# sdu-hpcl/BGSA

Measured on AMD Instinct MI355X. Metric: GCUPS (cell updates/sec) all-pairs Myers 150bp, higher is better.
Workload: dtype u32

## Files before the change

bgsa_amd/__init__.py:

```python
from __future__ import annotations

import ctypes
import os
import subprocess
from pathlib import Path

import numpy as np

HERE = Path(__file__).resolve().parent
LIB_PATH = Path(os.environ["BGSA_HIP_LIB"]) if os.environ.get("BGSA_HIP_LIB") else HERE / "libbgsa_hip.so"
LIB_AB_PATH = HERE / "libbgsa_hip_ab.so"
INCLUDE = HERE.parent / "include" / "bgsa_hip.h"

ALGO_MYERS, ALGO_BANDED, ALGO_BITPAL = 0, 1, 2
DISTANCE_BEYOND = -2
V_NUM = 64

_lib = None


class Params(ctypes.Structure):
    _fields_ = [("algo", ctypes.c_int), ("alignment", ctypes.c_int), ("match", ctypes.c_int),
                ("mismatch", ctypes.c_int), ("gap", ctypes.c_int), ("k", ctypes.c_int)]

# ... 96 lines not shown
            getattr(L, name).restype = restype
    L.bgsa_hip_stream_faults.argtypes = [i32]
    L.bgsa_hip_debug_inject_stream_fault.argtypes = [i32]
    L.bgsa_hip_set_auto_resident.argtypes = [i32]
    L.bgsa_hip_set_strict_resident.argtypes = [i32]
    L.bgsa_hip_stale_ranges.argtypes = [ctypes.POINTER(ctypes.c_uint64)]
    L.bgsa_hip_bucket_resident.argtypes = [vp, sz, i32]
    L.bgsa_hip_bucket_release.argtypes = [vp]
    u64p = ctypes.POINTER(ctypes.c_uint64)
    L.bgsa_hip_seam_stats.argtypes = [u64p, u64p, u64p]
    L.bgsa_hip_row_cache_stats.argtypes = [u64p, u64p]
    L.bgsa_hip_event_create.argtypes = [ctypes.POINTER(vp)]
    L.bgsa_hip_event_destroy.argtypes = [vp]
    L.bgsa_hip_event_record.argtypes = [vp, vp]
    L.bgsa_hip_event_synchronize.argtypes = [vp]
    L.bgsa_hip_event_elapsed_ms.argtypes = [vp, vp, ctypes.POINTER(ctypes.c_float)]
    L.bgsa_hip_stream_wait_event.argtypes = [vp, vp]
    L.bgsa_hip_query_stream.argtypes = [i32, vp, i32, i32, vp, i32]
    L.bgsa_hip_myers_band_stream.argtypes = [vp, i32, i32, vp, i32]
    L.bgsa_hip_myers_band_half.argtypes = [i32, i32]
    L.bgsa_hip_myers_band_stats.argtypes = [vp, i32]
    if hasattr(L, "bgsa_hip_myers_band_groups"):
        L.bgsa_hip_myers_band_groups.argtypes = [i32, i64, i32, i32, i32]
    L.bgsa_hip_kernel_name.argtypes = [i32, i32]
    L.bgsa_hip_kernel_name.restype = ctypes.c_char_p
    L.bgsa_hip_malloc.argtypes = [ctypes.POINTER(vp), sz]
    L.bgsa_hip_free.argtypes = [vp]
    L.bgsa_hip_malloc_host.argtypes = [ctypes.POINTER(vp), sz]
    L.bgsa_hip_free_host.argtypes = [vp]
    L.bgsa_hip_memcpy_h2d.argtypes = [vp, vp, sz, vp]
    L.bgsa_hip_memcpy_d2h.argtypes = [vp, vp, sz, vp]
    L.bgsa_hip_memset.argtypes = [vp, i32, sz, vp]
    L.bgsa_hip_stream_synchronize.argtypes = [vp]
    L.bgsa_hip_stream_create.argtypes = [ctypes.POINTER(vp)]
    L.bgsa_hip_stream_destroy.argtypes = [vp]
    L.bgsa_hip_set_device.argtypes = [i32]
    L.hip_handle_reads.argtypes = [vp, vp, i32, i64, i64]
    L.hip_handle_reads.restype = None
    L.hip_cal_align_score.argtypes = [vp, vp, vp, i32, i32, i32, i32, i32, i32, i32, i32, vp]
    L.hip_cal_align_score.restype = None
    L.align_hip.argtypes = [vp, vp, i32, i32, i32, i32, i32, vp, vp]
    L.align_hip.restype = None
    L.init_mapping_table.restype = None
    L.malloc_mem.argtypes = [ctypes.c_uint64]
    L.malloc_mem.restype = vp
    L.free_mem.argtypes = [vp]
# ... 726 lines not shown
```

bgsa_amd/csrc/bgsa_common.h:

```cpp
#pragma once

#include <hip/hip_runtime.h>
#include <stdint.h>
#include <stdlib.h>
#include <stdio.h>

#include <type_traits>

#include "../../include/bgsa_hip.h"

namespace bgsa {

constexpr int kLanes = HIP_V_NUM;
constexpr int kChars = BGSA_CHAR_NUM;
constexpr int kWavesPerBlock = 4;
constexpr int kMaxWords = 32;

void set_error(const char *what, hipError_t e, const char *file, int line);
void set_error_text(const char *text);

#define BGSA_HIP_TRY(expr)                                              \
    do {                                                                \
        hipError_t e_ = (expr);                                         \
        if (e_ != hipSuccess) {                                         \
// ... 39 lines not shown
        *n_blocks = (word_num + nw - 1) / nw;
        return nw;
    }
    template <typename F>
    static int dispatch(int nw, const char *family, F &&f)
    {
        int rc = BGSA_HIP_EUNSUPPORTED;
        if (((N == nw ? (rc = f(std::integral_constant<int, N>{}), true) : false) || ...)) return rc;
        char msg[128];
        snprintf(msg, sizeof msg, "%s: no kernel of %d words in this build", family, nw);
        set_error_text(msg);
        return BGSA_HIP_EUNSUPPORTED;
    }
    template <int M>
    constexpr Widths<N..., M> with() const { return {}; }
};
template <typename A, typename B> struct JoinWidths;
template <int... A, int... B> struct JoinWidths<Widths<A...>, Widths<B...>> { using type = Widths<A..., B...>; };
template <typename A, typename B> using Join = typename JoinWidths<A, B>::type;

int launch_myers(const ScoreArgs &a, int semi_global = 0);
const char *myers_kernel_name(int word_num, int semi_global = 0);
int myers_band_groups(int word_num, int64_t read_count, int ref_len, int read_len, int mixed_lengths);

constexpr int kCodeEnd = 5, kCodeRefill = 6;
inline int stream_windows(int ref_len) { return ref_len / 7 + 1; }
inline size_t stream_stride(int ref_len) { return static_cast<size_t>(stream_windows(ref_len) + 1) * 8; }
__host__ __device__ inline unsigned long long plain_stream_window(const char *row, int ref_len, int i)
{
    const int n_windows = ref_len / 7 + 1;
    unsigned long long win = 0;
    for (int j = 0; j < 8; j++) {
        unsigned code = kCodeEnd;
        if (i < n_windows) {
            const int pos = 7 * i + j;
            if (j == 7) code = (i < n_windows - 1) ? kCodeRefill : kCodeEnd;
            else if (pos < ref_len) {
                code = static_cast<unsigned char>(row[pos]);
                if (code > 4) code = 0;
            }
        }
        win |= static_cast<unsigned long long>(code) << (8 * j);
    }
    return win;
}
int launch_pack_queries(const char *d_content, int ref_len, int ref_start, int ref_end,
// ... 424 lines not shown
```

bgsa_amd/csrc/capi.hip:

```cpp
#include <stdlib.h>
#include <string.h>

#include <algorithm>
#include <atomic>
#include <chrono>
#include <map>
#include <memory>
#include <mutex>
#include <string>
#include <thread>
#include <utility>
#include <vector>

#include "bgsa_common.h"
#include "myers_band.h"

namespace bgsa {

static thread_local std::string g_last_error;

void set_error(const char *what, hipError_t e, const char *file, int line)
{
    char buf[512];
    snprintf(buf, sizeof buf, "%s failed: %s (%s:%d)", what, hipGetErrorString(e), file, line);
// ... 176 lines not shown
}

static size_t plan_workspace_bytes(const Plan &plan, int ref_len, int read_len, int n_queries)
{
    if (ref_len <= 0 || n_queries <= 0) return 0;
    const int algo = plan.kernel;
    if (read_len > 0 && plan_beyond_registers(plan, (read_len + 31) / 32)) {
        const int chains = algo == BGSA_ALGO_BITPAL ? plan.set->chains : 3;
        const size_t carries = (algo == BGSA_ALGO_BITPAL && plan.set->carry_words > 0)
                                   ? static_cast<size_t>(ref_len + 1) * plan.set->carry_words * kLanes * sizeof(uint32_t) * kWavesPerBlock * blocked_workgroups()
                                   : blocked_carry_bytes(ref_len, chains);
        const size_t blocked = static_cast<size_t>(blocked_stream_layout(ref_len, nullptr, nullptr)) * n_queries + 256 +
                               carries + 256;
#if BGSA_AB_KERNELS
        const char *ab = getenv(algo == BGSA_ALGO_BITPAL ? "BGSA_BITPAL_IMPL" : "BGSA_MYERS_IMPL");
        const size_t in_memory = (ab && ab[0] == 'c') ? long_state_bytes(algo, (read_len + 31) / 32) : 0;
        return blocked > in_memory ? blocked : in_memory;
#else
        return blocked;
#endif
    }
    if (algo == BGSA_ALGO_BANDED)
        return banded_stream_bound(ref_len) * n_queries + kTaskCounterBytes;
    return band_stream_stride(ref_len) * static_cast<size_t>(n_queries) + kTaskCounterBytes;
}

int ab_knob_refused(const char *what)
{
    std::string msg = std::string(what) + " selects a kernel that only the A/B flavour of the library carries: build it with `make -C "
                      "bgsa_amd/csrc ab` and point BGSA_HIP_LIB at libbgsa_hip_ab.so";
    set_error_text(msg.c_str());
    return BGSA_HIP_EUNSUPPORTED;
}

}

using namespace bgsa;

extern "C" {

int match_score = 0;
int mismatch_score = -1;
int gap_score = -1;
int dvdh_len = 16;
int full_bits = 1;
int threshold = HIP_BANDED_WORD_SIZE / 2 - 1;
int cpu_threads = 0;
// ... 301 lines not shown
        char msg[340];
        snprintf(msg, sizeof msg, "stream fault on device %d: flags 0x%x (%s%s%s%s) — at least one query was not scored", dev, value,
                 (value & BGSA_HIP_FAULT_BUDGET) ? "window budget exhausted before END " : "",
                 (value & BGSA_HIP_FAULT_CODE) ? "byte that is no stream code dispatched " : "",
                 (value & BGSA_HIP_FAULT_PAIR) ? "align_pairs / trace_pairs: query index outside [0, n_queries) " : "",
                 (value & BGSA_HIP_FAULT_BAND) ? "align_pairs_banded: a traceback step left its block's window" : "");
        set_error_text(msg);
    }
    return static_cast<int>(value);
}

int bgsa_hip_myers_band_half(int ref_len, int read_len)
{
    if (ref_len <= 0 || read_len <= 0) return BGSA_HIP_EINVAL;
    BandSchedule s;
    const int h = band_half(ref_len, read_len);
    return band_schedule(ref_len, read_len, h, (read_len + 31) / 32, &s) ? h : 0;
}

int bgsa_hip_myers_band_groups(int word_num, int64_t read_count, int ref_len, int read_len, int mixed_lengths)
{
    if (word_num <= 0 || read_count < 0 || ref_len <= 0 || read_len <= 0) return BGSA_HIP_EINVAL;
    return myers_band_groups(word_num, read_count, ref_len, read_len, mixed_lengths);
}

int bgsa_hip_myers_band_stream(const char *mapped_row, int ref_len, int read_len, unsigned char *dst, int cap)
{
    if (!mapped_row || ref_len <= 0 || read_len <= 0) return BGSA_HIP_EINVAL;
    BandSchedule s;
    if (!band_schedule(ref_len, read_len, band_half(ref_len, read_len), (read_len + 31) / 32, &s)) return 0;
    const int n = band_stream_layout(ref_len, s, mapped_row, nullptr);
    if (dst && cap >= n)
        for (int i = 0; 8 * i < n; i++) {
            memset(dst + 8 * i, kCodeEnd, 8);
            band_stream_layout(ref_len, s, mapped_row, dst + 8 * i, 8 * i, 8);
        }
    return n;
}

int bgsa_hip_myers_band_stats(unsigned long long *out, int clear)
{
    if (!out) return BGSA_HIP_EINVAL;
    out[0] = out[1] = 0;
    int dev = 0;
    unsigned *word = nullptr;
    if (int rc = existing_fault_word(&dev, &word)) return rc;
// ... 1126 lines not shown
```

bgsa_amd/csrc/myers_band.h:

```cpp
#pragma once

#include <stdlib.h>

#include "bgsa_common.h"

namespace bgsa {

constexpr int kBandMaxWords = 8;
constexpr int kBandMinWords = 3;
constexpr int kBandMaxSwitches = 2 * kBandMaxWords;
constexpr int kCodeSetWin = 7;
constexpr int kBandBadCode = 0xff;

struct BandSchedule {
    int n = 0;
    int row[kBandMaxSwitches] = {};
    int win[kBandMaxSwitches] = {};
};

__host__ __device__ inline int band_window_index(int nw, int a, int b) { return a * nw - a * (a - 1) / 2 + (b - a); }

inline int band_default_half(int len) { return (9 * len + 192) / 32; }

inline int band_half(int m, int n)
// ... 20 lines not shown
        const int a = (jlo - 1) / 32, b = (jhi - 1) / 32;
        words += b - a + 1;
        if (a != pa || b != pb) {
            if (s->n == kBandMaxSwitches) {
                s->n = 0;
                return false;
            }
            s->row[s->n] = i - 1;
            s->win[s->n] = band_window_index(nw, a, b);
            s->n++;
            pa = a;
            pb = b;
        }
    }
    if (5 * words > 4ll * m * nw) {
        s->n = 0;
        return false;
    }
    return true;
}

inline size_t band_stream_stride(int ref_len) { return stream_stride(ref_len + 3 * kBandMaxSwitches); }

__host__ __device__ inline int band_stream_layout(int len, const BandSchedule &s, const char *row, unsigned char *dst,
                                                  int first = 0, int count = 0x7fffffff)
{
    int pos = 0, sw = 0;
    auto in = [&]() { return dst && pos >= first && pos - first < count; };
    auto put = [&](int c) {
        if (in()) dst[pos - first] = static_cast<unsigned char>(c);
        pos++;
    };
    auto refill = [&]() {
        put(kCodeRefill);
        while (pos & 7) put(kCodeEnd);
    };
    for (int r = 0; r < len; r++) {
        if (dst && pos - first >= count) return pos;
        if (sw < s.n && s.row[sw] == r) {
            if ((pos & 7) >= 6) refill();
            put(kCodeSetWin);
            put(s.win[sw]);
            sw++;
        }
        if ((pos & 7) == 7) refill();
        if (in()) {
            const unsigned c = static_cast<unsigned char>(row[r]);
            dst[pos - first] = static_cast<unsigned char>(c > 4 ? 0u : c);
        }
        pos++;
    }
    if ((pos & 7) == 7) refill();
    put(kCodeEnd);
    while (pos & 7) put(kCodeEnd);
    for (int j = 0; j < 8; j++) put(kCodeEnd);
    return pos;
}

__host__ __device__ inline unsigned long long *band_launch_words(unsigned *task_counter)
{
    return reinterpret_cast<unsigned long long *>(task_counter + 16);
}

int launch_pack_band(const char *d_content, int ref_len, const BandSchedule &s, int ref_start, int ref_end, void *d_streams,
                     hipStream_t stream, unsigned *d_words);

__host__ __device__ inline unsigned long long *band_stats_words(unsigned *fault_word)
{
    return reinterpret_cast<unsigned long long *>(fault_word + 2);
}

}
```

bgsa_amd/csrc/myers_global.hip:

```cpp
#include <stdlib.h>
#include <string.h>

#include <algorithm>

#include "bgsa_common.h"
#include "myers_band.h"

namespace bgsa {

template <int NW, int G, bool SEMI = false>
__device__ __forceinline__ void myers_row(uint32_t (&vp)[G * NW], uint32_t (&vn)[G * NW],
                                          const uint32_t (&eq)[G * NW], int last_word = 0, int last_bit = 0,
                                          int *delta = nullptr)
{
#pragma unroll
  for (int gi = 0; gi < G; gi++) {
    uint32_t hp_prev = 0, hn_prev = 0;
    unsigned carry = 0;
#pragma unroll
    for (int ww = 0; ww < NW; ww++) {
        const int w = gi * NW + ww;
        const uint32_t pv = vp[w], mv = vn[w], e = eq[w];
        const uint32_t pm = e | mv;
        unsigned cout;
// ... 79 lines not shown
        }
#pragma unroll
        for (int gi = 0; gi < G; gi++) {
            int score = ref_len;
#pragma unroll
            for (int w = 0; w < NW; w++) {
                const int rem = read_len - 32 * w;
                const uint32_t m = rem >= 32 ? ~0u : (rem <= 0 ? 0u : ((1u << rem) - 1u));
                score += __popc(vp[gi * NW + w] & m) - __popc(vn[gi * NW + w] & m);
            }
            if (group0 + gi < n_groups)
                dst[static_cast<size_t>(q - ref_start) * ld + gi * kLanes] = static_cast<int16_t>(-score);
        }
    }
}

constexpr int kPeqMaxWords = 32;
constexpr int kSemiPeqMaxWords = 32;
constexpr int kPairMaxWords = 2;
constexpr int kBandPairMaxWords = 5;
#include "myers_rows_gen.inc"
#include "_gen/myers_band_rows_gen.inc"

template <int NW, int G, bool DYN = false, bool BAND = false, bool LENS = false>
__global__ __launch_bounds__(256) void myers_global_asm_kernel(
    const unsigned char *__restrict__ streams, const uint32_t *__restrict__ peq,
    int16_t *__restrict__ out, int ref_len, int read_len, long long ld, int n_groups, int word_num,
    int n_queries, int q_tile, int stream_stride_bytes, unsigned *__restrict__ fault_word,
    unsigned *__restrict__ task_counter, int band_limit = 0, unsigned long long *__restrict__ band_launch = nullptr,
    const int32_t *__restrict__ read_lens = nullptr)
{
    static_assert(!BAND || (NW >= kBandMinWords && NW <= kBandMaxWords && (G == 1 || (G == 2 && NW <= kBandPairMaxWords))),
                  "band: 3..8 words, one subject group per wave — or two up to 5 words");
    static_assert(!(LENS && BAND), "the certified band is derived from one (m, n): a length-aware launch runs full rows");
    constexpr bool kLenPerQuery = LENS && NW > 8;
    const int lane = threadIdx.x & (kLanes - 1);
    const unsigned wave_groups = (static_cast<unsigned>(n_groups) + G - 1) / G;
    const unsigned n_tasks = wave_groups * ((static_cast<unsigned>(n_queries) + q_tile - 1) / q_tile);
    unsigned task = 0, task_issued = 0;
    if constexpr (DYN) {
        task = first_wave_task();
        if (task >= n_tasks) return;
    }
    int band_on = 1, unreported = 0;
    do {
        int group0, tile;
        if constexpr (DYN) {
            group0 = static_cast<int>((task % wave_groups) * G);
            tile = static_cast<int>(task / wave_groups);
        } else {
            group0 = __builtin_amdgcn_readfirstlane((blockIdx.x * kWavesPerBlock + (threadIdx.x >> 6)) * G);
            tile = blockIdx.y;
            if (group0 >= n_groups) return;
        }

        uint32_t P[kChars][G * NW];
#pragma unroll
        for (int gi = 0; gi < G; gi++) {
            const bool live = group0 + gi < n_groups;
            const uint32_t *g = peq + static_cast<size_t>(group0 + gi) * kChars * word_num * kLanes + lane;
#pragma unroll
            for (int c = 0; c < kChars; c++)
#pragma unroll
                for (int w = 0; w < NW; w++)
                    P[c][gi * NW + w] = (live && w < word_num) ? g[(c * word_num + w) * kLanes] : 0u;
        }

        [[maybe_unused]] int own_len[G];
        if constexpr (LENS && !kLenPerQuery) {
#pragma unroll
            for (int gi = 0; gi < G; gi++)
                own_len[gi] = group0 + gi < n_groups ? lane_read_len(read_lens, static_cast<size_t>(group0 + gi) * kLanes + lane, read_len) : 0;
        }

        const int q0 = tile * q_tile;
        const int q1 = (q0 + q_tile < n_queries) ? q0 + q_tile : n_queries;
        int16_t *dst = out + static_cast<size_t>(group0) * kLanes + lane;

        for (int q = q0; q < q1; q++) {
            if constexpr (DYN) {
                if (q == q1 - 1) task_issued = issue_wave_task(task_counter);
            }
            uint32_t st[2 * G * NW];
#pragma unroll
            for (int w = 0; w < G * NW; w++) {
                st[2 * w] = ~0u;
                st[2 * w + 1] = 0u;
            }
            const unsigned long long s =
                reinterpret_cast<unsigned long long>(streams) + static_cast<unsigned long long>(q) * stream_stride_bytes;
            if constexpr (BAND) {
                const int n_live = G == 1 ? 1 : (group0 + 1 < n_groups ? 2 : 1);
                const int tried = band_on * n_live;
                int band = band_on, score[G];
                for (;;) {
                    const int left = myers_band_rows_asm<NW, G>(st, P, uniform_u64(s),
                                                                __builtin_amdgcn_readfirstlane(stream_stride_bytes / 8 - 2),
                                                                __builtin_amdgcn_readfirstlane(band));
                    note_stream_fault(fault_word, left);
#pragma unroll
                    for (int gi = 0; gi < G; gi++) {
                        score[gi] = ref_len;
#pragma unroll
                        for (int w = 0; w < NW; w++) {
                            const int rem = read_len - 32 * w;
                            const uint32_t m = rem >= 32 ? ~0u : (rem <= 0 ? 0u : ((1u << rem) - 1u));
                            score[gi] += __popc(st[2 * (gi * NW + w)] & m) - __popc(st[2 * (gi * NW + w) + 1] & m);
                        }
                    }
                    if (!band) break;
                    int n_over = 0;
#pragma unroll
                    for (int gi = 0; gi < G; gi++)
                        if (gi < n_live && __builtin_amdgcn_ballot_w64(score[gi] > band_limit) != 0) n_over++;
                    if (n_over == 0) break;
                    if constexpr (G == 1) n_over = 1;
                    band = 0;
                    unsigned long long r = static_cast<unsigned long long>(n_over),
                                       b = static_cast<unsigned long long>(unreported) + n_live;
                    if (lane == 0) {
                        r += atomicAdd(&band_launch[0], r);
                        b += atomicAdd(&band_launch[1], b);
                    }
                    r = uniform_u64(r);
                    b = uniform_u64(b);
                    unreported = -n_live;
                    if (b >= 64 && 8 * r > b) band_on = 0;
#pragma unroll
                    for (int w = 0; w < G * NW; w++) {
                        st[2 * w] = ~0u;
                        st[2 * w + 1] = 0u;
                    }
                }
                unreported += tried;
#pragma unroll
                for (int gi = 0; gi < G; gi++)
                    if (gi < n_live) dst[static_cast<size_t>(q) * ld + gi * kLanes] = static_cast<int16_t>(-score[gi]);
            } else {
                int left;
                if constexpr (NW <= kPairMaxWords)
// ... 387 lines not shown
    static const unsigned v = [] { const char *e = getenv("BGSA_MYERS_LDS_PAD"); return e ? static_cast<unsigned>(atoi(e)) : 0u; }();
    return v;
}

static int long_query_tile()
{
    static const int v = [] {
        const char *e = getenv("BGSA_MYERS_LONG_TILE");
        const int t = e ? atoi(e) : 32;
        return (t == 8 || t == 16 || t == 32) ? t : 32;
    }();
    return v;
}

bool peq_blocks()
{
    static const bool on = [] {
        const char *e = getenv("BGSA_MYERS_BLOCK_FORM");
        return !(e && strcmp(e, "planes") == 0);
    }();
    return on;
}

__global__ void band_stats_add_kernel(const unsigned long long *__restrict__ launch, unsigned long long *__restrict__ stats)
{
    atomicAdd(&stats[0], launch[0]);
    atomicAdd(&stats[1], launch[1]);
}

using AsmKernel = void (*)(const unsigned char *, const uint32_t *, int16_t *, int, int, long long, int, int, int, int, int,
                           unsigned *, unsigned *, int, unsigned long long *, const int32_t *);

template <int NW, int G>
int launch_asm(const ScoreArgs &a)
{
    const int nq = a.nq();
    constexpr bool kCounter = NW <= 8 || NW >= 30;
    constexpr bool kPairs = NW <= kPairMaxWords;
    constexpr bool kBandPair = G == 2 && !kPairs;
    static_assert(!kBandPair || NW <= kBandPairMaxWords, "two groups per wave: the pair kernels, or the band up to 5 words");
    const bool lens = a.d_read_lens != nullptr;
    const int64_t n_waves = (a.n_groups() + G - 1) / G;
    const TaskPlan plan = plan_tasks(nq, n_waves, static_cast<long long>(a.ref_len) * NW * G, NW >= 30 ? 8 : 32, kCounter,
                                     NW >= 30 ? long_query_tile() : query_tile_max(), lens);
    if (lens && kCounter && !plan.dynamic) {
        set_error_text("myers: too many tasks for one length-aware launch (split the query window)");
        return BGSA_HIP_EUNSUPPORTED;
    }
    note_query_tile(plan.q_tile);
    AsmKernel on_grid = nullptr, on_counter = nullptr;
    if constexpr (!kBandPair) {
        on_grid = myers_global_asm_kernel<NW, G, false>;
        if constexpr (kCounter) on_counter = myers_global_asm_kernel<NW, G, true>;
        if (lens) {
            if constexpr (kCounter) on_grid = nullptr, on_counter = myers_global_asm_kernel<NW, G, true, false, true>;
            else on_grid = myers_global_asm_kernel<NW, G, false, false, true>;
        }
    }
    BandSchedule sched;
    int h = 0;
    bool band = false;
    if constexpr ((G == 1 || kBandPair) && NW >= kBandMinWords && NW <= kBandMaxWords) {
        h = band_half(a.ref_len, a.read_len);
        band = !lens && band_schedule(a.ref_len, a.read_len, h, NW, &sched);
        if (band) {
            on_grid = myers_global_asm_kernel<NW, G, false, true>;
            on_counter = myers_global_asm_kernel<NW, G, true, true>;
        }
    }
    if (kBandPair && !band) {
        set_error_text("myers: two subject groups per wave selected for a launch without the certified band");
        return BGSA_HIP_EUNSUPPORTED;
    }
    const int stride = static_cast<int>(band ? band_stream_stride(a.ref_len) : kPairs ? pair_stream_stride(a.ref_len) : stream_stride(a.ref_len));
    unsigned *words = task_counter_in(a.d_workspace, static_cast<size_t>(stride) * nq);
    LaunchGrid lg;
    if (int rc = plan_grid(plan, n_waves, nq, words,
                           [&] { return on_counter ? persistent_blocks_for(on_counter, myers_lds_pad()) : persistent_blocks(); }, "myers", &lg))
        return rc;
    if (int rc = band     ? launch_pack_band(a.d_content, a.ref_len, sched, a.ref_start, a.ref_end, a.d_workspace, a.stream, words)
                 : kPairs ? launch_pack_query_pairs(a.d_content, a.ref_len, a.ref_start, a.ref_end, a.d_workspace, a.stream, lg.counter)
                          : launch_pack_queries(a.d_content, a.ref_len, a.ref_start, a.ref_end, a.d_workspace, a.stream, lg.counter))
        return rc;
    unsigned *fault = nullptr;
    if (int rc = stream_guard(a.d_workspace, stride, kPairs ? kPairRefill : kCodeRefill, band ? kBandBadCode : kPairs ? -1 : 7, a.stream, &fault))
        return rc;
    unsigned long long *guard = band ? band_launch_words(words) : nullptr;
    const AsmKernel kernel = lg.counter ? on_counter : on_grid;
    hipLaunchKernelGGL(kernel, lg.grid, dim3(256), lg.counter ? myers_lds_pad() : 0u, a.stream,
                       static_cast<const unsigned char *>(a.d_workspace), a.d_peq, a.results<int16_t>(), a.ref_len, a.read_len,
                       static_cast<long long>(a.read_count), static_cast<int>(a.n_groups()), a.word_num, nq, plan.q_tile, stride,
                       fault, lg.counter, band ? 2 * h + 1 : 0, guard, a.d_read_lens);
    BGSA_HIP_TRY(hipGetLastError());
    if (band) {
        hipLaunchKernelGGL(band_stats_add_kernel, dim3(1), dim3(1), 0, a.stream, static_cast<const unsigned long long *>(guard),
                           band_stats_words(fault));
        BGSA_HIP_TRY(hipGetLastError());
    }
    return BGSA_HIP_OK;
}

template <int NW>
int launch_semi_asm(const ScoreArgs &a)
{
    const int nq = a.nq(), stride = static_cast<int>(stream_stride(a.ref_len));
    const int q_tile = pick_q_tile(nq, a.n_groups(), a.ref_len, NW);
    note_query_tile(q_tile);
    LaunchGrid lg;
    if (int rc = plan_grid({q_tile, false}, a.n_groups(), nq, nullptr, no_counter_kernel, "myers", &lg)) return rc;
    if (int rc = launch_pack_queries(a.d_content, a.ref_len, a.ref_start, a.ref_end, a.d_workspace, a.stream)) return rc;
    unsigned *fault = nullptr;
    if (int rc = stream_guard(a.d_workspace, stride, kCodeRefill, 7, a.stream, &fault)) return rc;
    hipLaunchKernelGGL((myers_semi_asm_kernel<NW>), lg.grid, dim3(256), 0, a.stream,
                       static_cast<const unsigned char *>(a.d_workspace), a.d_peq, a.results<int16_t>(), a.ref_len,
                       a.read_len, static_cast<long long>(a.read_count), static_cast<int>(a.n_groups()), a.word_num,
// ... 155 lines not shown
            c.G = 2;
        }
    } else if (semi && word_num > myers_semi_max_plain_words()) {
        c.family = MyersFamily::kBlockedPeq;
        c.nw = PeqBlockWidths::pick_blocks(word_num, &c.n_blocks);
    } else if (semi) {
        c.family = MyersFamily::kSemiPlanes;
        c.nw = SemiPlanesWidths::pick(word_num);
    } else {
        c.family = MyersFamily::kPlanes;
        c.nw = Join<PlanesAbWidths, PlanesWidths>::pick(word_num);
        if (!PlanesWidths::has(c.nw)) c.refused = ab_only("BGSA_MYERS_PEQ_MAX_WORDS");
    }
    return c;
}

}

int myers_band_groups(int word_num, int64_t read_count, int ref_len, int read_len, int mixed_lengths)
{
    if (word_num < 1 || word_num > kMaxWords) return 1;
    const MyersChoice c = myers_select(word_num, 0, read_count, ref_len, read_len, mixed_lengths != 0);
    return c.family == MyersFamily::kAsmBandPairs ? 2 : 1;
}

const char *myers_kernel_name(int word_num, int semi_global)
{
    static thread_local char name[64];
    const MyersChoice c = myers_select(word_num, semi_global, 2 * kLanes);
    switch (c.family) {
    case MyersFamily::kAsm:
    case MyersFamily::kAsmBandPairs:
    case MyersFamily::kAsmPairs: snprintf(name, sizeof name, "myers_global_asm_kernel<%d, %d>", c.nw, c.G); break;
    case MyersFamily::kSemiAsm: snprintf(name, sizeof name, "myers_semi_asm_kernel<%d>", c.nw); break;
    case MyersFamily::kPlanes: snprintf(name, sizeof name, "myers_global_planes_kernel<%d>", c.nw); break;
    case MyersFamily::kSemiPlanes: snprintf(name, sizeof name, "myers_semi_planes_kernel<%d>", c.nw); break;
    case MyersFamily::kStateInMemory:
        snprintf(name, sizeof name, peq_blocks() ? "myers_blocked_kernel<%d, true>" : "myers_blocked_kernel<%d>", c.nw);
        break;
    case MyersFamily::kBlockedPeq: snprintf(name, sizeof name, c.semi ? "myers_blocked_kernel<%d, true, true>" : "myers_blocked_kernel<%d, true>", c.nw); break;
    case MyersFamily::kBlockedPlanes: snprintf(name, sizeof name, "myers_blocked_kernel<%d>", c.nw); break;
    case MyersFamily::kCompiler: snprintf(name, sizeof name, c.semi ? "myers_global_kernel<%d, 1, true>" : "myers_global_kernel<%d, 1>", c.nw); break;
    }
    return name;
}

// ... 50 lines not shown
```

bgsa_amd/csrc/preprocess.hip:

```cpp
#include <algorithm>
#include <thread>
#include <vector>

#include "bgsa_common.h"
#include "myers_band.h"

namespace bgsa {

__host__ __device__ __forceinline__ uint32_t map_char(uint32_t ch)
{
    return ch == 'C' ? 1u : ch == 'G' ? 2u : ch == 'T' ? 3u : ch == 'N' ? 4u : 0u;
}


__global__ __launch_bounds__(256) void preprocess_global_kernel(const char *__restrict__ rows,
                                                                uint32_t *__restrict__ peq, int len,
                                                                long long read_count, int word_num,
                                                                int data_bits)
{
    const long long subject = static_cast<long long>(blockIdx.x) * blockDim.x + threadIdx.x;
    if (subject >= read_count) return;
    const long long group = subject >> 6;
    const int lane = static_cast<int>(subject & 63);
    const char *row = rows + subject * (len + 1);
// ... 186 lines not shown
    if (tid >= static_cast<long long>(n_queries) * per) return;
    const int q = static_cast<int>(tid / per), i = static_cast<int>(tid % per);
    unsigned char win[8];
    for (int j = 0; j < 8; j++) win[j] = kCodeEnd;
    band_stream_layout(len, sched, content + static_cast<size_t>(ref_start + q) * (len + 1), win, 8 * i, 8);
    unsigned long long w = 0;
    for (int j = 0; j < 8; j++) w |= static_cast<unsigned long long>(win[j]) << (8 * j);
    streams[tid] = w;
}

int launch_pack_band(const char *d_content, int ref_len, const BandSchedule &s, int ref_start, int ref_end, void *d_streams,
                     hipStream_t stream, unsigned *d_words)
{
    const int nq = ref_end - ref_start;
    if (nq <= 0) return BGSA_HIP_OK;
    const int stride = static_cast<int>(band_stream_stride(ref_len));
    if (band_stream_layout(ref_len, s, nullptr, nullptr) > stride) {
        set_error_text("myers band: stream longer than its stride");
        return BGSA_HIP_EINVAL;
    }
    const long long total = static_cast<long long>(nq) * (stride / 8);
    hipLaunchKernelGGL(pack_band_kernel, dim3(static_cast<unsigned>((total + 255) / 256)), dim3(256), 0, stream, d_content,
                       static_cast<unsigned long long *>(d_streams), ref_len, s, ref_start, nq, stride / 8, d_words);
    BGSA_HIP_TRY(hipGetLastError());
    return BGSA_HIP_OK;
}

__global__ __launch_bounds__(64) void pack_blocked_kernel(const char *__restrict__ content,
                                                          unsigned char *__restrict__ streams, int len,
                                                          int ref_start, int n_queries, int stride)
{
    const int q = blockIdx.x * blockDim.x + threadIdx.x;
    if (q >= n_queries) return;
    blocked_stream_layout(len, content + static_cast<size_t>(ref_start + q) * (len + 1),
                          streams + static_cast<size_t>(q) * stride);
}

int launch_pack_blocked(const char *d_content, int len, int ref_start, int ref_end, void *d_streams,
                        hipStream_t stream)
{
    const int nq = ref_end - ref_start;
    if (nq <= 0) return BGSA_HIP_OK;
    const int stride = blocked_stream_layout(len, nullptr, nullptr);
    hipLaunchKernelGGL(pack_blocked_kernel, dim3((nq + 63) / 64), dim3(64), 0, stream, d_content,
                       static_cast<unsigned char *>(d_streams), len, ref_start, nq, stride);
    BGSA_HIP_TRY(hipGetLastError());
// ... 107 lines not shown
```

bgsa_amd/csrc/rows_ir.py:

```python
#!/usr/bin/env python3
from __future__ import annotations

from dataclasses import dataclass, field

import numpy as np


def tt(fn) -> int:
    return fn(0xF0, 0xCC, 0xAA) & 0xFF


TT_XOR3 = tt(lambda a, b, c: a ^ b ^ c)
TT_MAJ = tt(lambda a, b, c: (a & b) | (a & c) | (b & c))
TT_OR3 = tt(lambda a, b, c: a | b | c)
TT_NOR3 = tt(lambda a, b, c: ~(a | b | c))


@dataclass
class Op:
    kind: str
    dst: str = ""
    srcs: tuple = ()
    imm: int = 0
    dst2: str = ""
# ... 510 lines not shown
    def refill():
        out.append(6)
        while len(out) % 8:
            out.append(5)

    def put(c):
        if len(out) % 8 == 7:
            refill()
        out.append(c)

    cur = None
    for i in range(m):
        if win[i] != cur:
            if len(out) % 8 >= 6:
                refill()
            out += bytes([7, myers_window_index(nw, *win[i])])
            cur = win[i]
        put(int(codes[i]))
    put(5)
    while len(out) % 8:
        out.append(5)
    out += bytes([5] * 8)
    return bytes(out)


def run_band_stream(nw: int, state: list, peq: np.ndarray, stream: bytes, band: bool = True, balanced: bool = False,
                    schedule=None, groups: int = 1) -> int:
    windows = [(a, b) for a in range(nw) for b in range(a, nw)]
    bodies = {}
    cur = (0, nw - 1)
    pos, rows = 0, 0
    while True:
        c = stream[pos]
        if c == 5:
            return rows
        if c == 6:
            pos = (pos | 7) + 1
            continue
        if c == 7:
            k = stream[pos + 1]
            assert k < len(windows) and myers_window_index(nw, *windows[k]) == k
            cur = windows[k] if band else (0, nw - 1)
            pos += 2
            continue
        assert c < 5
        if cur not in bodies:
# ... 1478 lines not shown
```

include/bgsa_hip.h:

```cpp
#ifndef BGSA_HIP_H
#define BGSA_HIP_H

#include <stddef.h>
#include <stdint.h>

#ifdef __cplusplus
extern "C" {
#endif

#define BGSA_CHAR_NUM 5
#define HIP_V_NUM 64
#define HIP_WORD_SIZE 32
#define HIP_BANDED_WORD_SIZE 64
#define HIP_MAX_ERROR 127
typedef uint32_t hip_read_t;
typedef uint32_t hip_data_t;
typedef int16_t hip_write_t;
typedef int8_t hip_banded_write_t;

#ifndef BGSA_HAVE_SEQ_T
#define BGSA_HAVE_SEQ_T
typedef struct _seq_t {
    int len;
    int64_t size;
// ... 194 lines not shown
int64_t bgsa_hip_reference_window_count(int64_t ref_len, int window_len, int stride);
int64_t bgsa_hip_reference_window_start(int64_t ref_len, int window_len, int stride, int64_t window);
int bgsa_hip_reference_windows_dev(const char *d_reference, int64_t ref_len, int window_len, int stride,
                                   const int32_t *d_window_ids, int64_t first_id, int64_t n_rows,
                                   char *d_content, void *stream);
int bgsa_hip_reference_placements_dev(int64_t ref_len, int window_len, int stride,
                                      const int32_t *d_hit_windows, int64_t n_reads, int k,
                                      const int32_t *d_span, const int32_t *d_n_ops, int32_t *d_cigar, int cigar_cap,
                                      int32_t *d_strand, int64_t *d_ref_begin, int64_t *d_ref_end, int32_t *d_keep,
                                      void *stream);

#define BGSA_HIP_FAULT_BUDGET 1
#define BGSA_HIP_FAULT_CODE 2
#define BGSA_HIP_FAULT_PAIR 4
#define BGSA_HIP_FAULT_BAND 8
int bgsa_hip_stream_faults(int clear);
int bgsa_hip_debug_inject_stream_fault(int kind);

int bgsa_hip_clock_probe_start(int n_probes, unsigned max_ms, void *caller_stream);
int bgsa_hip_clock_probe_stop(double *mhz, int *xcc, int cap, int *n_out, double *seconds);

int bgsa_hip_query_stream(int algo, const char *mapped_row, int ref_len, int k, unsigned char *dst, int cap);

int bgsa_hip_myers_band_stream(const char *mapped_row, int ref_len, int read_len, unsigned char *dst, int cap);
int bgsa_hip_myers_band_half(int ref_len, int read_len);
int bgsa_hip_myers_band_groups(int word_num, int64_t read_count, int ref_len, int read_len, int mixed_lengths);
int bgsa_hip_myers_band_stats(unsigned long long *out, int clear);

int bgsa_hip_last_query_tile(void);

const char *bgsa_hip_kernel_name(int algo, int word_num);

#ifdef __cplusplus
}
#endif
#endif
```

Before: 390,300.

## Share Myers band prefix rows across sorted queries via LDS checkpoints

```diff
diff --git a/bgsa_amd/__init__.py b/bgsa_amd/__init__.py
--- a/bgsa_amd/__init__.py
+++ b/bgsa_amd/__init__.py
@@ -142,6 +142,9 @@
     L.bgsa_hip_myers_band_stats.argtypes = [vp, i32]
     if hasattr(L, "bgsa_hip_myers_band_groups"):
         L.bgsa_hip_myers_band_groups.argtypes = [i32, i64, i32, i32, i32]
+    if hasattr(L, "bgsa_hip_myers_prefix_depths"):
+        L.bgsa_hip_myers_prefix_depths.argtypes = [i32, i64, i32, i32, i32, i32, ip, i32]
+        L.bgsa_hip_myers_band_segments.argtypes = [vp, i32, i32, ip, i32, vp, i32, ip]
     L.bgsa_hip_kernel_name.argtypes = [i32, i32]
     L.bgsa_hip_kernel_name.restype = ctypes.c_char_p
     L.bgsa_hip_malloc.argtypes = [ctypes.POINTER(vp), sz]
diff --git a/bgsa_amd/csrc/bgsa_common.h b/bgsa_amd/csrc/bgsa_common.h
--- a/bgsa_amd/csrc/bgsa_common.h
+++ b/bgsa_amd/csrc/bgsa_common.h
@@ -85,6 +85,7 @@
 int launch_myers(const ScoreArgs &a, int semi_global = 0);
 const char *myers_kernel_name(int word_num, int semi_global = 0);
 int myers_band_groups(int word_num, int64_t read_count, int ref_len, int read_len, int mixed_lengths);
+int myers_prefix_depths(int word_num, int64_t read_count, int ref_len, int read_len, int n_queries, int mixed_lengths, int *depths);
 
 constexpr int kCodeEnd = 5, kCodeRefill = 6;
 inline int stream_windows(int ref_len) { return ref_len / 7 + 1; }
diff --git a/bgsa_amd/csrc/capi.hip b/bgsa_amd/csrc/capi.hip
--- a/bgsa_amd/csrc/capi.hip
+++ b/bgsa_amd/csrc/capi.hip
@@ -222,7 +222,7 @@
     }
     if (algo == BGSA_ALGO_BANDED)
         return banded_stream_bound(ref_len) * n_queries + kTaskCounterBytes;
-    return band_stream_stride(ref_len) * static_cast<size_t>(n_queries) + kTaskCounterBytes;
+    return band_segments_stride_bound(ref_len) * static_cast<size_t>(n_queries) + kTaskCounterBytes + prefix_order_bytes(n_queries);
 }
 
 int ab_knob_refused(const char *what)
@@ -570,6 +570,40 @@
 {
     if (word_num <= 0 || read_count < 0 || ref_len <= 0 || read_len <= 0) return BGSA_HIP_EINVAL;
     return myers_band_groups(word_num, read_count, ref_len, read_len, mixed_lengths);
+}
+
+int bgsa_hip_myers_prefix_depths(int word_num, int64_t read_count, int ref_len, int read_len, int n_queries, int mixed_lengths,
+                                 int *depths, int cap)
+{
+    if (word_num <= 0 || read_count < 0 || ref_len <= 0 || read_len <= 0 || n_queries < 0 || cap < 0 || (cap > 0 && !depths)) return BGSA_HIP_EINVAL;
+    int d[kPrefixMaxDepths] = {};
+    const int n = myers_prefix_depths(word_num, read_count, ref_len, read_len, n_queries, mixed_lengths, d);
+    for (int j = 0; j < n && j < cap; j++) depths[j] = d[j];
+    return n;
+}
+
+int bgsa_hip_myers_band_segments(const char *mapped_row, int ref_len, int read_len, const int *depths, int n_depths,
+                                 unsigned char *dst, int cap, int *offsets)
+{
+    if (!mapped_row || ref_len <= 0 || read_len <= 0 || !depths || n_depths < 1 || n_depths > kPrefixMaxDepths) return 0;
+    BandSchedule s;
+    if (!band_schedule(ref_len, read_len, band_half(ref_len, read_len), (read_len + 31) / 32, &s)) return 0;
+    PrefixPlan p;
+    p.n = n_depths;
+    for (int j = 0; j < n_depths; j++) p.depth[j] = depths[j];
+    if (!prefix_plan_layout(ref_len, (read_len + 31) / 32, s, &p)) return 0;
+    const int n = p.off[p.n + 1];
+    if (offsets)
+        for (int j = 0; j <= p.n + 1; j++) offsets[j] = p.off[j];
+    if (dst && cap >= n)
+        for (int i = 0; i < n / 8; i++) {
+            int seg = 0;
+            while (seg < p.n && p.off[seg + 1] <= 8 * i) seg++;
+            for (int j = 0; j < 8; j++) dst[8 * i + j] = kCodeEnd;
+            band_rows_layout(s, seg ? p.depth[seg - 1] : 0, seg < p.n ? p.depth[seg] : ref_len, seg == p.n, mapped_row, dst + 8 * i,
+                             8 * i - p.off[seg], 8);
+        }
+    return n;
 }
 
 int bgsa_hip_myers_band_stream(const char *mapped_row, int ref_len, int read_len, unsigned char *dst, int cap)
diff --git a/bgsa_amd/csrc/myers_band.h b/bgsa_amd/csrc/myers_band.h
--- a/bgsa_amd/csrc/myers_band.h
+++ b/bgsa_amd/csrc/myers_band.h
@@ -66,8 +66,8 @@
 
 inline size_t band_stream_stride(int ref_len) { return stream_stride(ref_len + 3 * kBandMaxSwitches); }
 
-__host__ __device__ inline int band_stream_layout(int len, const BandSchedule &s, const char *row, unsigned char *dst,
-                                                  int first = 0, int count = 0x7fffffff)
+__host__ __device__ inline int band_rows_layout(const BandSchedule &s, int r0, int r1, bool spare, const char *row, unsigned char *dst,
+                                                int first = 0, int count = 0x7fffffff)
 {
     int pos = 0, sw = 0;
     auto in = [&]() { return dst && pos >= first && pos - first < count; };
@@ -79,9 +79,10 @@
         put(kCodeRefill);
         while (pos & 7) put(kCodeEnd);
     };
-    for (int r = 0; r < len; r++) {
+    while (sw + 1 < s.n && s.row[sw + 1] <= r0) sw++;
+    for (int r = r0; r < r1; r++) {
         if (dst && pos - first >= count) return pos;
-        if (sw < s.n && s.row[sw] == r) {
+        if (sw < s.n && (s.row[sw] == r || r == r0)) {
             if ((pos & 7) >= 6) refill();
             put(kCodeSetWin);
             put(s.win[sw]);
@@ -97,9 +98,65 @@
     if ((pos & 7) == 7) refill();
     put(kCodeEnd);
     while (pos & 7) put(kCodeEnd);
-    for (int j = 0; j < 8; j++) put(kCodeEnd);
+    for (int j = 0; spare && j < 8; j++) put(kCodeEnd);
     return pos;
 }
+
+__host__ __device__ inline int band_stream_layout(int len, const BandSchedule &s, const char *row, unsigned char *dst,
+                                                  int first = 0, int count = 0x7fffffff)
+{
+    return band_rows_layout(s, 0, len, true, row, dst, first, count);
+}
+
+constexpr int kPrefixMaxDepths = 5;
+constexpr int kPrefixKeyChars = 10;
+struct PrefixPlan {
+    int n = 0;
+    int depth[kPrefixMaxDepths] = {};
+    int off[kPrefixMaxDepths + 2] = {};
+};
+inline size_t band_segments_stride_bound(int ref_len) { return band_stream_stride(ref_len) + 16 * kPrefixMaxDepths; }
+
+inline bool prefix_plan_layout(int m, int nw, const BandSchedule &s, PrefixPlan *p)
+{
+    const int n = p->n;
+    p->n = 0;
+    if (n < 1 || n > kPrefixMaxDepths || s.n < 1) return false;
+    for (int j = 0; j < n; j++)
+        if (p->depth[j] < 1 || p->depth[j] > kPrefixKeyChars || p->depth[j] >= m || (j && p->depth[j] <= p->depth[j - 1])) return false;
+    for (int i = 0; i < s.n && s.row[i] < p->depth[n - 1]; i++)
+        if (s.win[i] != band_window_index(nw, 0, 0) && s.win[i] != band_window_index(nw, 0, 1)) return false;
+    int pos = 0;
+    for (int j = 0; j <= n; j++) {
+        p->off[j] = pos;
+        pos += band_rows_layout(s, j ? p->depth[j - 1] : 0, j < n ? p->depth[j] : m, j == n, nullptr, nullptr);
+    }
+    p->off[n + 1] = pos;
+    if (static_cast<size_t>(pos) > band_segments_stride_bound(m) || pos / 8 > 255) return false;
+    p->n = n;
+    return true;
+}
+
+struct PrefixEntry {
+    int q;
+    short lcp, seg;
+};
+inline size_t prefix_order_bytes(int n_queries) { return static_cast<size_t>(n_queries) * (sizeof(PrefixEntry) + sizeof(uint32_t)) + 256; }
+__host__ __device__ inline PrefixEntry *prefix_entries(unsigned *task_counter)
+{
+    return reinterpret_cast<PrefixEntry *>(reinterpret_cast<unsigned char *>(task_counter) + kTaskCounterBytes);
+}
+inline unsigned long long prefix_segments_word(const PrefixPlan &p)
+{
+    unsigned long long w = static_cast<unsigned long long>(p.n) << 56;
+    for (int j = 0; j <= p.n && p.n; j++) w |= static_cast<unsigned long long>(p.off[j] / 8) << (8 * j);
+    return w;
+}
+
+int launch_prefix_order(const char *d_content, int ref_len, int ref_start, int ref_end, int q_tile, const PrefixPlan &p,
+                        unsigned *d_words, hipStream_t stream);
+int launch_pack_band_segments(const char *d_content, int ref_len, const BandSchedule &s, const PrefixPlan &p, int ref_start,
+                              int ref_end, void *d_streams, hipStream_t stream, unsigned *d_words);
 
 __host__ __device__ inline unsigned long long *band_launch_words(unsigned *task_counter)
 {
diff --git a/bgsa_amd/csrc/myers_global.hip b/bgsa_amd/csrc/myers_global.hip
--- a/bgsa_amd/csrc/myers_global.hip
+++ b/bgsa_amd/csrc/myers_global.hip
@@ -125,17 +125,26 @@
 #include "myers_rows_gen.inc"
 #include "_gen/myers_band_rows_gen.inc"
 
-template <int NW, int G, bool DYN = false, bool BAND = false, bool LENS = false>
-__global__ __launch_bounds__(256) void myers_global_asm_kernel(
+extern __shared__ uint4 prefix_slots[];
+constexpr int band_kernel_waves(int nw, int g, bool dyn, bool share)
+{
+    if (!share) return 1;
+    if (g == 2) return nw == 3 ? 8 : (nw == 4 ? (dyn ? 6 : 7) : 5);
+    return nw <= 5 ? 8 : (nw == 6 ? (dyn ? 7 : 8) : (nw == 7 ? (dyn ? 6 : 7) : (dyn ? 5 : 6)));
+}
+template <int NW, int G, bool DYN = false, bool BAND = false, bool LENS = false, bool SHARE = false>
+__global__ __launch_bounds__(256) __attribute__((amdgpu_waves_per_eu(band_kernel_waves(NW, G, DYN, SHARE)))) void myers_global_asm_kernel(
     const unsigned char *__restrict__ streams, const uint32_t *__restrict__ peq,
     int16_t *__restrict__ out, int ref_len, int read_len, long long ld, int n_groups, int word_num,
     int n_queries, int q_tile, int stream_stride_bytes, unsigned *__restrict__ fault_word,
     unsigned *__restrict__ task_counter, int band_limit = 0, unsigned long long *__restrict__ band_launch = nullptr,
-    const int32_t *__restrict__ read_lens = nullptr)
+    const int32_t *__restrict__ read_lens = nullptr, unsigned long long prefix_segments = 0,
+    const PrefixEntry *__restrict__ order = nullptr)
 {
     static_assert(!BAND || (NW >= kBandMinWords && NW <= kBandMaxWords && (G == 1 || (G == 2 && NW <= kBandPairMaxWords))),
                   "band: 3..8 words, one subject group per wave — or two up to 5 words");
     static_assert(!(LENS && BAND), "the certified band is derived from one (m, n): a length-aware launch runs full rows");
+    static_assert(!SHARE || BAND, "prefix sharing: the band kernels only");
     constexpr bool kLenPerQuery = LENS && NW > 8;
     const int lane = threadIdx.x & (kLanes - 1);
     const unsigned wave_groups = (static_cast<unsigned>(n_groups) + G - 1) / G;
@@ -180,9 +189,15 @@
         const int q1 = (q0 + q_tile < n_queries) ? q0 + q_tile : n_queries;
         int16_t *dst = out + static_cast<size_t>(group0) * kLanes + lane;
 
-        for (int q = q0; q < q1; q++) {
+        for (int k = q0; k < q1; k++) {
             if constexpr (DYN) {
-                if (q == q1 - 1) task_issued = issue_wave_task(task_counter);
+                if (k == q1 - 1) task_issued = issue_wave_task(task_counter);
+            }
+            int q = k, seg = 0;
+            if constexpr (SHARE) {
+                const int2 e = *reinterpret_cast<const int2 *>(order + k);
+                q = __builtin_amdgcn_readfirstlane(e.x);
+                seg = __builtin_amdgcn_readfirstlane(e.y >> 16);
             }
             uint32_t st[2 * G * NW];
 #pragma unroll
@@ -196,11 +211,34 @@
                 const int n_live = G == 1 ? 1 : (group0 + 1 < n_groups ? 2 : 1);
                 const int tried = band_on * n_live;
                 int band = band_on, score[G];
+                const int n_depths = SHARE ? static_cast<int>(prefix_segments >> 56) : 0;
+                const bool sharing = SHARE && band_on;
+                [[maybe_unused]] uint4 *const slots = prefix_slots + ((threadIdx.x >> 6) * G) * kLanes + lane;
+                if (!sharing) seg = 0;
+                if (SHARE && seg) {
+#pragma unroll
+                    for (int gi = 0; gi < G; gi++) {
+                        const uint4 v = slots[((seg - 1) * kWavesPerBlock * G + gi) * kLanes];
+                        st[2 * gi * NW] = v.x;
+                        st[2 * gi * NW + 1] = v.y;
+                        st[2 * gi * NW + 2] = v.z;
+                        st[2 * gi * NW + 3] = v.w;
+                    }
+                }
                 for (;;) {
-                    const int left = myers_band_rows_asm<NW, G>(st, P, uniform_u64(s),
-                                                                __builtin_amdgcn_readfirstlane(stream_stride_bytes / 8 - 2),
-                                                                __builtin_amdgcn_readfirstlane(band));
-                    note_stream_fault(fault_word, left);
+                    for (; seg <= n_depths; seg++) {
+                        const int at = SHARE ? static_cast<int>((prefix_segments >> (8 * seg)) & 0xffu) * 8 : 0;
+                        const int left = myers_band_rows_asm<NW, G>(st, P, uniform_u64(s + static_cast<unsigned>(at)),
+                                                                    __builtin_amdgcn_readfirstlane((stream_stride_bytes - at) / 8 - 2),
+                                                                    __builtin_amdgcn_readfirstlane(band));
+                        note_stream_fault(fault_word, left);
+                        if (SHARE && sharing && band && seg < n_depths) {
+#pragma unroll
+                            for (int gi = 0; gi < G; gi++)
+                                slots[(seg * kWavesPerBlock * G + gi) * kLanes] =
+                                    make_uint4(st[2 * gi * NW], st[2 * gi * NW + 1], st[2 * gi * NW + 2], st[2 * gi * NW + 3]);
+                        }
+                    }
 #pragma unroll
                     for (int gi = 0; gi < G; gi++) {
                         score[gi] = ref_len;
@@ -219,6 +257,7 @@
                     if (n_over == 0) break;
                     if constexpr (G == 1) n_over = 1;
                     band = 0;
+                    seg = 0;
                     unsigned long long r = static_cast<unsigned long long>(n_over),
                                        b = static_cast<unsigned long long>(unreported) + n_live;
                     if (lane == 0) {
@@ -652,6 +691,61 @@
     return on;
 }
 
+constexpr bool kPrefixShareDefault = true;
+constexpr int kPrefixMinQueries = 2000;
+constexpr int kPrefixMinTile = 16;
+struct PrefixKnob {
+    int mode;
+    int n, depth[kPrefixMaxDepths];
+};
+static const PrefixKnob &prefix_knob()
+{
+    static const PrefixKnob k = [] {
+        PrefixKnob v = {kPrefixShareDefault ? 1 : 0, 0, {}};
+        const char *e = getenv("BGSA_MYERS_PREFIX_SHARE");
+        if (!e || !*e) return v;
+        if (!strchr(e, ',')) {
+            const int d = atoi(e);
+            if (d <= 0) v.mode = 0;
+            else if (d == 1) v.mode = 1;
+            else v = {2, 1, {d}};
+            return v;
+        }
+        v = {2, 0, {}};
+        for (const char *c = e; c; c = strchr(c, ',') ? strchr(c, ',') + 1 : nullptr) {
+            if (v.n == kPrefixMaxDepths) return PrefixKnob{0, 0, {}};
+            v.depth[v.n++] = atoi(c);
+        }
+        return v;
+    }();
+    return k;
+}
+
+void prefix_select(int ref_len, int nw, const BandSchedule &s, int nq, int q_tile, int64_t read_count, PrefixPlan *p)
+{
+    *p = PrefixPlan{};
+    const PrefixKnob &knob = prefix_knob();
+    if (knob.mode == 0 || q_tile < kPrefixMinTile || nq < kPrefixMinTile || nq > 8 * read_count) return;
+    PrefixPlan want;
+    if (knob.mode == 2) {
+        want.n = knob.n;
+        for (int j = 0; j < knob.n; j++) want.depth[j] = knob.depth[j];
+    } else {
+        if (nq < kPrefixMinQueries) return;
+        int d0 = 0;
+        for (long long v = nq; v >= 4; v /= 4) d0++;
+        for (int d = d0 - 1; d <= d0 + 1; d++)
+            if (d >= 1 && d <= kPrefixKeyChars && d < ref_len) want.depth[want.n++] = d;
+        while (want.n > 0) {
+            PrefixPlan probe = want;
+            if (prefix_plan_layout(ref_len, nw, s, &probe)) break;
+            want.n--;
+        }
+    }
+    if (prefix_plan_layout(ref_len, nw, s, &want)) *p = want;
+}
+size_t prefix_lds_bytes(const PrefixPlan &p, int groups) { return static_cast<size_t>(p.n) * kWavesPerBlock * groups * kLanes * sizeof(uint4); }
+
 __global__ void band_stats_add_kernel(const unsigned long long *__restrict__ launch, unsigned long long *__restrict__ stats)
 {
     atomicAdd(&stats[0], launch[0]);
@@ -659,7 +753,7 @@
 }
 
 using AsmKernel = void (*)(const unsigned char *, const uint32_t *, int16_t *, int, int, long long, int, int, int, int, int,
-                           unsigned *, unsigned *, int, unsigned long long *, const int32_t *);
+                           unsigned *, unsigned *, int, unsigned long long *, const int32_t *, unsigned long long, const PrefixEntry *);
 
 template <int NW, int G>
 int launch_asm(const ScoreArgs &a)
@@ -688,6 +782,7 @@
         }
     }
     BandSchedule sched;
+    PrefixPlan prefix;
     int h = 0;
     bool band = false;
     if constexpr ((G == 1 || kBandPair) && NW >= kBandMinWords && NW <= kBandMaxWords) {
@@ -696,19 +791,32 @@
         if (band) {
             on_grid = myers_global_asm_kernel<NW, G, false, true>;
             on_counter = myers_global_asm_kernel<NW, G, true, true>;
+            prefix_select(a.ref_len, NW, sched, nq, plan.q_tile, a.read_count, &prefix);
+            if (prefix.n) {
+                on_grid = myers_global_asm_kernel<NW, G, false, true, false, true>;
+                on_counter = myers_global_asm_kernel<NW, G, true, true, false, true>;
+            }
         }
     }
     if (kBandPair && !band) {
         set_error_text("myers: two subject groups per wave selected for a launch without the certified band");
         return BGSA_HIP_EUNSUPPORTED;
     }
-    const int stride = static_cast<int>(band ? band_stream_stride(a.ref_len) : kPairs ? pair_stream_stride(a.ref_len) : stream_stride(a.ref_len));
+    const unsigned lds = (plan.dynamic ? myers_lds_pad() : 0u) + static_cast<unsigned>(prefix_lds_bytes(prefix, G));
+    const int stride = static_cast<int>(prefix.n  ? static_cast<size_t>(prefix.off[prefix.n + 1])
+                                        : band    ? band_stream_stride(a.ref_len)
+                                        : kPairs  ? pair_stream_stride(a.ref_len)
+                                                  : stream_stride(a.ref_len));
     unsigned *words = task_counter_in(a.d_workspace, static_cast<size_t>(stride) * nq);
     LaunchGrid lg;
     if (int rc = plan_grid(plan, n_waves, nq, words,
-                           [&] { return on_counter ? persistent_blocks_for(on_counter, myers_lds_pad()) : persistent_blocks(); }, "myers", &lg))
+                           [&] { return on_counter ? persistent_blocks_for(on_counter, lds) : persistent_blocks(); }, "myers", &lg))
         return rc;
-    if (int rc = band     ? launch_pack_band(a.d_content, a.ref_len, sched, a.ref_start, a.ref_end, a.d_workspace, a.stream, words)
+    if (prefix.n)
+        if (int rc = launch_prefix_order(a.d_content, a.ref_len, a.ref_start, a.ref_end, plan.q_tile, prefix, words, a.stream))
+            return rc;
+    if (int rc = prefix.n ? launch_pack_band_segments(a.d_content, a.ref_len, sched, prefix, a.ref_start, a.ref_end, a.d_workspace, a.stream, words)
+                 : band   ? launch_pack_band(a.d_content, a.ref_len, sched, a.ref_start, a.ref_end, a.d_workspace, a.stream, words)
                  : kPairs ? launch_pack_query_pairs(a.d_content, a.ref_len, a.ref_start, a.ref_end, a.d_workspace, a.stream, lg.counter)
                           : launch_pack_queries(a.d_content, a.ref_len, a.ref_start, a.ref_end, a.d_workspace, a.stream, lg.counter))
         return rc;
@@ -717,10 +825,11 @@
         return rc;
     unsigned long long *guard = band ? band_launch_words(words) : nullptr;
     const AsmKernel kernel = lg.counter ? on_counter : on_grid;
-    hipLaunchKernelGGL(kernel, lg.grid, dim3(256), lg.counter ? myers_lds_pad() : 0u, a.stream,
+    hipLaunchKernelGGL(kernel, lg.grid, dim3(256), lds, a.stream,
                        static_cast<const unsigned char *>(a.d_workspace), a.d_peq, a.results<int16_t>(), a.ref_len, a.read_len,
                        static_cast<long long>(a.read_count), static_cast<int>(a.n_groups()), a.word_num, nq, plan.q_tile, stride,
-                       fault, lg.counter, band ? 2 * h + 1 : 0, guard, a.d_read_lens);
+                       fault, lg.counter, band ? 2 * h + 1 : 0, guard, a.d_read_lens, prefix_segments_word(prefix),
+                       static_cast<const PrefixEntry *>(prefix_entries(words)));
     BGSA_HIP_TRY(hipGetLastError());
     if (band) {
         hipLaunchKernelGGL(band_stats_add_kernel, dim3(1), dim3(1), 0, a.stream, static_cast<const unsigned long long *>(guard),
@@ -922,6 +1031,21 @@
     if (word_num < 1 || word_num > kMaxWords) return 1;
     const MyersChoice c = myers_select(word_num, 0, read_count, ref_len, read_len, mixed_lengths != 0);
     return c.family == MyersFamily::kAsmBandPairs ? 2 : 1;
+}
+
+int myers_prefix_depths(int word_num, int64_t read_count, int ref_len, int read_len, int n_queries, int mixed_lengths, int *depths)
+{
+    if (word_num < 1 || word_num > kMaxWords || n_queries < 1) return 0;
+    const MyersChoice c = myers_select(word_num, 0, read_count, ref_len, read_len, mixed_lengths != 0);
+    if ((c.family != MyersFamily::kAsm && c.family != MyersFamily::kAsmBandPairs) || mixed_lengths) return 0;
+    BandSchedule sched;
+    if (!band_schedule(ref_len, read_len, band_half(ref_len, read_len), c.nw, &sched)) return 0;
+    const int64_t n_waves = (read_count / kLanes + c.G - 1) / c.G;
+    const TaskPlan plan = plan_tasks(n_queries, n_waves, static_cast<long long>(ref_len) * c.nw * c.G, 32, true, query_tile_max());
+    PrefixPlan p;
+    prefix_select(ref_len, c.nw, sched, n_queries, plan.q_tile, read_count, &p);
+    for (int j = 0; j < p.n; j++) depths[j] = p.depth[j];
+    return p.n;
 }
 
 const char *myers_kernel_name(int word_num, int semi_global)
diff --git a/bgsa_amd/csrc/preprocess.hip b/bgsa_amd/csrc/preprocess.hip
--- a/bgsa_amd/csrc/preprocess.hip
+++ b/bgsa_amd/csrc/preprocess.hip
@@ -232,6 +232,110 @@
     const long long total = static_cast<long long>(nq) * (stride / 8);
     hipLaunchKernelGGL(pack_band_kernel, dim3(static_cast<unsigned>((total + 255) / 256)), dim3(256), 0, stream, d_content,
                        static_cast<unsigned long long *>(d_streams), ref_len, s, ref_start, nq, stride / 8, d_words);
+    BGSA_HIP_TRY(hipGetLastError());
+    return BGSA_HIP_OK;
+}
+
+__global__ __launch_bounds__(256) void prefix_key_kernel(const char *__restrict__ content, int len, int ref_start, int n_queries,
+                                                         uint32_t *__restrict__ keys)
+{
+    const int q = blockIdx.x * blockDim.x + threadIdx.x;
+    if (q >= n_queries) return;
+    const char *row = content + static_cast<size_t>(ref_start + q) * (len + 1);
+    uint32_t key = 0;
+    for (int j = 0; j < kPrefixKeyChars; j++) {
+        const unsigned c = j < len ? static_cast<unsigned char>(row[j]) : 0u;
+        key = (key << 3) | (c > 4 ? 0u : c);
+    }
+    keys[q] = key;
+}
+__global__ __launch_bounds__(256) void prefix_rank_kernel(const uint32_t *__restrict__ keys, int n_queries,
+                                                          PrefixEntry *__restrict__ entries)
+{
+    __shared__ uint32_t block_keys[256];
+    const int q = blockIdx.x * blockDim.x + threadIdx.x;
+    const uint32_t own = q < n_queries ? keys[q] : 0u;
+    int rank = 0;
+    for (int base = 0; base < n_queries; base += 256) {
+        block_keys[threadIdx.x] = base + static_cast<int>(threadIdx.x) < n_queries ? keys[base + threadIdx.x] : ~0u;
+        __syncthreads();
+        for (int j = 0; j < 256; j++) {
+            const uint32_t other = block_keys[j];
+            rank += (other < own || (other == own && base + j < q)) ? 1 : 0;
+        }
+        __syncthreads();
+    }
+    if (q < n_queries) entries[rank].q = q;
+}
+__global__ __launch_bounds__(256) void prefix_lcp_kernel(const uint32_t *__restrict__ keys, int n_queries, int q_tile, PrefixPlan plan,
+                                                         PrefixEntry *__restrict__ entries)
+{
+    const int k = blockIdx.x * blockDim.x + threadIdx.x;
+    if (k >= n_queries) return;
+    int lcp = 0;
+    if (k % q_tile) {
+        const uint32_t diff = keys[entries[k].q] ^ keys[entries[k - 1].q];
+        lcp = diff ? (3 * kPrefixKeyChars - 1 - (31 - __clz(diff))) / 3 : kPrefixKeyChars;
+        if (lcp > plan.depth[plan.n - 1]) lcp = plan.depth[plan.n - 1];
+    }
+    int seg = 0;
+    while (seg < plan.n && plan.depth[seg] <= lcp) seg++;
+    entries[k].lcp = static_cast<short>(lcp);
+    entries[k].seg = static_cast<short>(seg);
+}
+
+int launch_prefix_order(const char *d_content, int ref_len, int ref_start, int ref_end, int q_tile, const PrefixPlan &p,
+                        unsigned *d_words, hipStream_t stream)
+{
+    const int nq = ref_end - ref_start;
+    if (nq <= 0 || p.n < 1) return BGSA_HIP_OK;
+    PrefixEntry *entries = prefix_entries(d_words);
+    uint32_t *keys = reinterpret_cast<uint32_t *>(entries + nq);
+    const dim3 grid((nq + 255) / 256), block(256);
+    hipLaunchKernelGGL(prefix_key_kernel, grid, block, 0, stream, d_content, ref_len, ref_start, nq, keys);
+    BGSA_HIP_TRY(hipGetLastError());
+    hipLaunchKernelGGL(prefix_rank_kernel, grid, block, 0, stream, static_cast<const uint32_t *>(keys), nq, entries);
+    BGSA_HIP_TRY(hipGetLastError());
+    hipLaunchKernelGGL(prefix_lcp_kernel, grid, block, 0, stream, static_cast<const uint32_t *>(keys), nq, q_tile, p, entries);
+    BGSA_HIP_TRY(hipGetLastError());
+    return BGSA_HIP_OK;
+}
+
+__global__ __launch_bounds__(256) void pack_band_segments_kernel(const char *__restrict__ content, unsigned long long *__restrict__ streams,
+                                                                 int len, BandSchedule sched, PrefixPlan plan, int ref_start,
+                                                                 int n_queries, int per, unsigned *__restrict__ words)
+{
+    const long long tid = static_cast<long long>(blockIdx.x) * blockDim.x + threadIdx.x;
+    if (tid == 0) {
+        words[0] = 0u;
+        band_launch_words(words)[0] = band_launch_words(words)[1] = 0ull;
+    }
+    if (tid >= static_cast<long long>(n_queries) * per) return;
+    const int q = static_cast<int>(tid / per), i = static_cast<int>(tid % per);
+    int seg = 0;
+    while (seg < plan.n && plan.off[seg + 1] <= 8 * i) seg++;
+    unsigned char win[8];
+    for (int j = 0; j < 8; j++) win[j] = kCodeEnd;
+    band_rows_layout(sched, seg ? plan.depth[seg - 1] : 0, seg < plan.n ? plan.depth[seg] : len, seg == plan.n,
+                     content + static_cast<size_t>(ref_start + q) * (len + 1), win, 8 * i - plan.off[seg], 8);
+    unsigned long long w = 0;
+    for (int j = 0; j < 8; j++) w |= static_cast<unsigned long long>(win[j]) << (8 * j);
+    streams[tid] = w;
+}
+
+int launch_pack_band_segments(const char *d_content, int ref_len, const BandSchedule &s, const PrefixPlan &p, int ref_start,
+                              int ref_end, void *d_streams, hipStream_t stream, unsigned *d_words)
+{
+    const int nq = ref_end - ref_start;
+    if (nq <= 0) return BGSA_HIP_OK;
+    const int stride = p.off[p.n + 1];
+    if (p.n < 1 || stride <= 0 || (stride & 7) || static_cast<size_t>(stride) > band_segments_stride_bound(ref_len)) {
+        set_error_text("myers band: segmented stream longer than its stride");
+        return BGSA_HIP_EINVAL;
+    }
+    const long long total = static_cast<long long>(nq) * (stride / 8);
+    hipLaunchKernelGGL(pack_band_segments_kernel, dim3(static_cast<unsigned>((total + 255) / 256)), dim3(256), 0, stream, d_content,
+                       static_cast<unsigned long long *>(d_streams), ref_len, s, p, ref_start, nq, stride / 8, d_words);
     BGSA_HIP_TRY(hipGetLastError());
     return BGSA_HIP_OK;
 }
diff --git a/bgsa_amd/csrc/rows_ir.py b/bgsa_amd/csrc/rows_ir.py
--- a/bgsa_amd/csrc/rows_ir.py
+++ b/bgsa_amd/csrc/rows_ir.py
@@ -556,6 +556,39 @@
         out.append(5)
     out += bytes([5] * 8)
     return bytes(out)
+
+
+def myers_band_segments(codes, m: int, n: int, h: int, nw: int, depths) -> tuple[bytes, list] | None:
+    win = myers_band_windows(m, n, h, nw)
+    depths = list(depths)
+    if win is None or not depths or depths != sorted(set(depths)) or depths[0] < 1 or depths[-1] >= m:
+        return None
+    if any(w not in ((0, 0), (0, 1)) for w in win[:depths[-1]]):
+        return None
+    out, offsets = bytearray(), []
+    cuts = [0] + depths + [m]
+    for j in range(len(cuts) - 1):
+        offsets.append(len(out))
+        seg = bytearray()
+        cur = None
+        for i in range(cuts[j], cuts[j + 1]):
+            if win[i] != cur:
+                if len(seg) % 8 >= 6:
+                    seg += bytes([6] + [5] * (7 - len(seg) % 8))
+                seg += bytes([7, myers_window_index(nw, *win[i])])
+                cur = win[i]
+            if len(seg) % 8 == 7:
+                seg.append(6)
+            seg.append(int(codes[i]))
+        if len(seg) % 8 == 7:
+            seg.append(6)
+        seg.append(5)
+        seg += bytes([5] * (-len(seg) % 8))
+        if j == len(cuts) - 2:
+            seg += bytes([5] * 8)
+        out += seg
+    offsets.append(len(out))
+    return bytes(out), offsets
 
 
 def run_band_stream(nw: int, state: list, peq: np.ndarray, stream: bytes, band: bool = True, balanced: bool = False,
diff --git a/include/bgsa_hip.h b/include/bgsa_hip.h
--- a/include/bgsa_hip.h
+++ b/include/bgsa_hip.h
@@ -240,6 +240,10 @@
 
 int bgsa_hip_query_stream(int algo, const char *mapped_row, int ref_len, int k, unsigned char *dst, int cap);
 
+int bgsa_hip_myers_prefix_depths(int word_num, int64_t read_count, int ref_len, int read_len, int n_queries, int mixed_lengths,
+                                 int *depths, int cap);
+int bgsa_hip_myers_band_segments(const char *mapped_row, int ref_len, int read_len, const int *depths, int n_depths,
+                                 unsigned char *dst, int cap, int *offsets);
 int bgsa_hip_myers_band_stream(const char *mapped_row, int ref_len, int read_len, unsigned char *dst, int cap);
 int bgsa_hip_myers_band_half(int ref_len, int read_len);
 int bgsa_hip_myers_band_groups(int word_num, int64_t read_count, int ref_len, int read_len, int mixed_lengths);
```

Result: faster. 394,400, median of 6 (+1.0%).
